# m-hamza-mughal/convofusion

Hardware: AMD Instinct MI355X
Metric: denoise-steps/sec (B=32 per GPU, 196-token latent, 1500 audio tokens, 1000-step DDPM schedule) (higher is better)
Workload: dtype f16x3 (fp16 hi/lo split operands, 3 MFMAs per product, f32 accumulate; f32-equivalent); fused cross-attention against the long (audio) memory: single-f16 operands (keys, values, queries, probabilities), f32 accumulate, in DDPM runs (operand policy 15; 1000-step DDPM golden at this shape: 2.3e-5 from; 1 GPU; configs[1]: B=32/GPU synthetic, L=196, S=(32, 1500, 32, 8, 1), 7-way guidance (denoiser batch 224), DDPM 1000-step schedule, 20 timed iterations of the hipGraph-captured loop; parallelism=batch-shard x1, one all_gather of latents

## Files before the change

convofusion_amd/csrc/cfd_dev.hip:

```cpp
#include "cfd_internal.hpp"

extern "C" int cfd_debug_stop_stage(cfd_handle c, int stage) {
  if (!c) return fail(CFD_E_ARG, "null handle");
  c->stop_stage = stage;
  return CFD_OK;
}

extern "C" int cfd_debug_weg_stop(cfd_handle c, int stop) {
  if (!c) return fail(CFD_E_ARG, "null handle");
  if (stop != 0) {
    if (!c->rt_on || !c->weg_rt_on) return fail(CFD_E_STATE, "cfd_debug_weg_stop: this handle does not evaluate on the row-tile path");
    const int l = stop / 16, k = stop % 16;
    const bool ok = stop > 0 && ((l < c->nl && k >= 1 && k <= 9 && !(l == c->nl - 1 && k < 5)) || stop == 10);
    if (!ok) return fail(CFD_E_ARG, "cfd_debug_weg_stop: %d names no launch of the reverse sweep (16 l + k, k = 1 .. 9; the top layer has no B1 .. B4; 10 = the embedding)", stop);
  }
  c->wrt.stop = stop;
  return CFD_OK;
}

static int weg_debug_buffer(Ctx* c, const char* what, float** p, size_t* n) {
  WegRtState& s = c->wrt;
  if (s.sig.empty() || !s.B) return fail(CFD_E_STATE, "'%s': no row-tile WEG evaluation has run on this handle", what);
  const size_t M = (size_t)s.B * s.L;
  int l = -1, k = -1;
// ... 27 lines not shown
    HIPCHK(hipMemcpy(p, v.data(), n * 4, hipMemcpyHostToDevice));
  }
  return CFD_OK;
}

extern "C" int cfd_debug_read(cfd_handle c, const char* what, float* dst_dev, size_t numel) {
  if (!c || !what || !dst_dev) return fail(CFD_E_ARG, "null argument");
  HIPCHK(hipSetDevice(c->cfg.device));
  if (!strcmp(what, "setup_launches")) {
    const float f = (float)c->setup_launches;
    HIPCHK(hipMemcpy(dst_dev, &f, 4, hipMemcpyHostToDevice));
    return CFD_OK;
  }
  if (!strcmp(what, "sat")) {
    unsigned int n[2] = {0, 0};
    HIPCHK(hipDeviceSynchronize());
    HIPCHK(hipMemcpy(n, c->sat.p, 8, hipMemcpyDeviceToHost));
    const float f = (float)n[0] + (float)n[1];
    HIPCHK(hipMemcpy(dst_dev, &f, 4, hipMemcpyHostToDevice));
    return CFD_OK;
  }
#if RT_STAMP
  if (!strcmp(what, "rt_ring")) {
    HIPCHK(hipDeviceSynchronize());
    if (numel * 4 < sizeof(unsigned long long) * 4 * 4096 + 8) return fail(CFD_E_ARG, "rt_ring needs %zu bytes", sizeof(unsigned long long) * 4 * 4096 + 8);
    HIPCHK(hipMemcpyFromSymbol(dst_dev, HIP_SYMBOL(g_rt_ring), sizeof(unsigned long long) * 4 * 4096, 0, hipMemcpyDeviceToDevice));
    HIPCHK(hipMemcpyFromSymbol(reinterpret_cast<char*>(dst_dev) + sizeof(unsigned long long) * 4 * 4096, HIP_SYMBOL(g_rt_seq), 4, 0, hipMemcpyDeviceToDevice));
    return CFD_OK;
  }
#endif
  if (!strcmp(what, "weg.info")) {
    if (numel < 5) return fail(CFD_E_ARG, "weg.info needs 5 floats");
    const float f[5] = {(float)c->wrt.launches, (float)c->wrt.Sp_tot, (float)c->wrt.dy_keys, (float)c->wrt.focus_large, (float)c->wrt.stop_gi};
    HIPCHK(hipMemcpy(dst_dev, f, sizeof(f), hipMemcpyHostToDevice));
    return CFD_OK;
  }
  if (!strncmp(what, "weg.", 4)) {
    float* p = nullptr;
    size_t n = 0;
    CHK(weg_debug_buffer(c, what, &p, &n));
    if (numel > n) return fail(CFD_E_ARG, "buffer '%s' holds %zu floats, asked for %zu", what, n, numel);
    HIPCHK(hipDeviceSynchronize());
    HIPCHK(hipMemcpy(dst_dev, p, numel * 4, hipMemcpyDeviceToDevice));
    return CFD_OK;
  }
  const DBuf* b = nullptr;
  if (!strcmp(what, "x")) b = &c->w->x;
  else if (!strcmp(what, "temb")) b = &c->w->temb_tab;
  else if (!strcmp(what, "ss")) b = &c->w->ss_tab;
  else if (!strcmp(what, "eps")) b = &c->w->eps;
  else if (!strcmp(what, "sc")) b = &c->w->sc;
  else if (!strcmp(what, "ssc")) b = &c->w->ssc;
  else if (!strcmp(what, "xa_stamps")) b = &c->w->xa_stamps;
  else return fail(CFD_E_ARG, "unknown buffer '%s'", what);
  if (numel * 4 > b->bytes) return fail(CFD_E_ARG, "buffer '%s' holds %zu bytes, asked for %zu", what, b->bytes, numel * 4);
  HIPCHK(hipDeviceSynchronize());
  HIPCHK(hipMemcpy(dst_dev, b->p, numel * 4, hipMemcpyDeviceToDevice));
  return CFD_OK;
}
```

convofusion_amd/csrc/cfd_internal.hpp:

```cpp
#pragma once
#include <hip/hip_runtime.h>

#include <cmath>
#include <cstdarg>
#include <cstdio>
#include <cstdlib>
#include <cstring>
#include <algorithm>
#include <map>
#include <string>
#include <vector>

#include "../../include/cfdenoise.h"
#include "../../include/cfdenoise_dev.h"
#include "gemm_sp.hpp"
#include "rows.hpp"
#include "attn_fused.hpp"
#include "xattn_fused.hpp"
#include "rowtile.hpp"


int fail(int code, const char* fmt, ...);
#define HIPCHK(expr)                                                                               \
  do {                                                                                             \
// ... 10 lines not shown

struct DBuf {
  void* p = nullptr;
  size_t bytes = 0;
  int ensure(size_t n) {
    if (n <= bytes) return CFD_OK;
    if (p) (void)hipFree(p);
    p = nullptr;
    bytes = 0;
    HIPCHK(hipMalloc(&p, n));
    bytes = n;
    return CFD_OK;
  }
  void release() {
    if (p) (void)hipFree(p);
    p = nullptr;
    bytes = 0;
  }
  template <class T> T* as() const { return reinterpret_cast<T*>(p); }
};

struct LayerW {
  DBuf wqkv_sp, bqk, wo_sp, bo2, wtb1_sp, wtb2_sp, w1_sp, w2_sp, cross_bias;
  DBuf wqk_f, wv_f, w1_f, ln_cd;
  const float *ln1g, *ln1b, *tb1g, *tb1b, *btb1, *ln2g, *ln2b, *tb2g, *tb2b, *btb2, *ln3g, *ln3b, *b1, *b2;
};

struct Problem {
  int Be = 0, L = 0, Lp = 0;
  long long M = 0;
  int U[CFD_NMEM], S[CFD_NMEM], Sp[CFD_NMEM], off[CFD_NMEM], Sp_tot = 0;
  const float* mem[CFD_NMEM];
  const int* map[CFD_NMEM];
  const uint8_t* mask[CFD_NMEM];
  int has_mask[CFD_NMEM];
  float* att[CFD_NMEM];
  int att_b0 = 0, att_nb = 0;
  bool prev_same = false;
  bool att_fused = false;
  long long att_slot[CFD_NMEM] = {0, 0, 0, 0, 0};
  int tmode = 0;
  int lv_rows = 0, lv_i0 = 0, lv_U[CFD_NMEM] = {0, 0, 0, 0, 0};
  int share_B = 0;
  int T = 1;
  int jbig = -1, nruns = 0, nlong = 0, nshort = 0;
  int run_row0[8], run_len[8], run_u[8];
  int xa_nwg = 0;
  int xa0_nwg_a = 0, xa0_nwg_b = 0;
  bool xa_flush = false;
  int xa_one = -1;
  bool xa_f16 = false;
  int xa_f16_mask = 0;
  int static_mask = 0;
  bool rt = false;
  int rt_use_inst = 0;
  unsigned char rt_inst[CFD_NMEM][RT_ARG_ROWS];
};

struct RtSave {
  float* x[CFD_MAX_LAYERS + 1][5];
  char* qk[CFD_MAX_LAYERS];
  char* vt[CFD_MAX_LAYERS];
  float* sc[CFD_MAX_LAYERS];
  float* cst[CFD_MAX_LAYERS];
  float* pre[CFD_MAX_LAYERS];
};

struct WegRtState {
  std::vector<long long> sig;
  RtSave sv;
  float *att = nullptr, *d_att = nullptr, *fws = nullptr, *dP = nullptr, *G[3] = {nullptr, nullptr, nullptr}, *dz = nullptr, *dy = nullptr,
        *dh = nullptr, *dO = nullptr, *dqkv = nullptr;
  int launches = 0;
  int T = 1;
  int stop = 0, stop_gi = -1;
  int B = 0, L = 0, Sp_tot = 0, St = 0;
  int dy_keys = 0, focus_large = 0;
};

struct Work {
  Problem pb;
  DBuf x, h_sp, qkv_sp, vts_sp, ssc, sp_sp, o_sp, u_sp, sc, p_sp, eps, sample_sp;
  DBuf ln_stat;
  DBuf n_sp[CFD_NMEM], kall_sp[CFD_NMEM], cb[CFD_NMEM], vt_all[CFD_NMEM];
  DBuf temb_tab, h1_tab, ss_tab, trows, iota, long_rows, short_rows, zero_mask;
  DBuf ca[CFD_NMEM], asq[CFD_NMEM], kbtab[CFD_NMEM], vbtab[CFD_NMEM], b_tab, b_sp, bsq, zeros512;
  DBuf xa_wgs, xa_segs, xa_stamps, xa0_wgs_a, xa0_segs_a, xa0_wgs_b, xa0_segs_b, xa_dedup, xa_one_va, xa_att_raw, xa_att_mc, xa_att_fin, xa_att_desc;
  DBuf d_step;
  bool fwd_mem_valid = false;
  int fwd_U[CFD_NMEM] = {0, 0, 0, 0, 0}, fwd_S[CFD_NMEM] = {0, 0, 0, 0, 0}, fwd_Be = 0, fwd_L = 0;
  bool fwd_att = false;
  bool fwd_mask[CFD_NMEM] = {false, false, false, false, false}, fwd_map[CFD_NMEM] = {false, false, false, false, false};
  unsigned long long fwd_wver = 0;
  DBuf rt_vt, rt_cbt[CFD_NMEM];
  DBuf k16[CFD_NMEM], v16[CFD_NMEM];
  DBuf rt_cur;
  std::vector<int32_t> tt_key;
  long long tt_wver = -1;
  int tt_mem_mask = 0;
  const float* now_ss = nullptr;
  const float* now_kb[CFD_NMEM] = {nullptr, nullptr, nullptr, nullptr, nullptr};
  const float* now_vb[CFD_NMEM] = {nullptr, nullptr, nullptr, nullptr, nullptr};
  void release() {
    DBuf* all[] = {&x, &h_sp, &qkv_sp, &vts_sp, &ssc, &sp_sp, &o_sp, &u_sp, &sc, &p_sp, &eps, &sample_sp, &temb_tab, &h1_tab, &ss_tab, &trows, &iota,
                   &long_rows, &short_rows, &zero_mask, &ln_stat, &b_tab, &b_sp, &bsq, &zeros512, &xa_wgs, &xa_segs, &xa_stamps, &xa0_wgs_a, &xa0_segs_a, &xa0_wgs_b, &xa0_segs_b, &xa_dedup, &xa_one_va, &xa_att_raw, &xa_att_mc, &xa_att_fin, &xa_att_desc, &d_step, &rt_vt, &rt_cur};
    for (DBuf* b : all) b->release();
    for (int j = 0; j < CFD_NMEM; ++j) {
      n_sp[j].release(); kall_sp[j].release(); cb[j].release(); vt_all[j].release(); ca[j].release(); asq[j].release(); kbtab[j].release();
      vbtab[j].release(); rt_cbt[j].release(); k16[j].release(); v16[j].release();
    }
  }
};

struct RunMode {
  bool weighted = false;
  int k0 = 0;
  bool edit = false;
  float* traj = nullptr;
  bool anchor = false;
  const float* anchor_ring = nullptr;
  int anchor_n = 0;
  bool tie = false;
  bool tie_final = false;
  bool replay = false;
};

struct cfd_handle_s {
  cfd_config cfg;
  int nl = 0;
  bool finalized = false;
  std::map<std::string, DBuf> raw;
  std::map<std::string, size_t> raw_numel;
  DBuf we_sp, wp_sp, we_all, be_all;
  DBuf wp_f, ln_cd_p;
  DBuf wk_all_sp[CFD_NMEM], wv_all_sp[CFD_NMEM];
  std::vector<LayerW> lw;
  int qpe_rows = 0, mpe_rows = 0;
  DBuf tsin;
  int tsin_rows = 0;
  Work wk[2];
  Work* w = &wk[0];
  long long wver = 0;
  int setup_launches = 0;
  DBuf sat;
  bool memside_in_forward = false;
  bool run_counts = false;
  DBuf acen;
  bool acen_on = false, acen_valid = false, acen_measured = false;
  int acen_hits = 0;
  float acen_tau = 0.f;
  unsigned int* sat_mem() const { return sat.as<unsigned int>() + CFD_SAT_MEM; }
  unsigned int* sat_in() const { return sat.as<unsigned int>() + CFD_SAT_IN; }
  bool want_f16 = false;
  bool hint_same_mem = false;
  bool hint_now = false;
  bool census_pending = false;
  bool rt_on = true, weg_rt_on = true, weg_graph_on = true, fused_xattn = true, l0_dedup = true, share0 = true, permute = true;
  long long rt_max_rows = 700;
// ... 131 lines not shown
}

template <int CFD_KI = 0>
__global__ void replicate_rows_kernel(float4* x, long long n4, int G) {
  const long long i = (long long)blockIdx.x * blockDim.x + threadIdx.x;
  if (i >= n4) return;
  const float4 v = x[i];
  for (int g = 1; g < G; ++g) x[(long long)g * n4 + i] = v;
}

template <int CFD_KI = 0>
__global__ void fill_f32_kernel(float* p, long long n, float v) {
  const long long i = (long long)blockIdx.x * blockDim.x + threadIdx.x;
  if (i < n) p[i] = v;
}


template <int CFD_KI = 0, int PRED = 0>
__global__ void sched_step_kernel(const float* eps, const float* noise, float* x, size_t n, StepCoef c, int kind, int clip, float* x0_out) {
  const size_t i = (size_t)blockIdx.x * blockDim.x + threadIdx.x;
  if (i >= n) return;
  const float e = eps[i], xv = x[i];
  const float x0 = step_x0_of<PRED>(c, clip, xv, e);
  if (x0_out) x0_out[i] = x0;
  float prev = (kind == 0) ? c.c0 * x0 + c.cx * xv : c.c0 * x0 + c.cx * step_eps_of<PRED>(c, xv, e);
  if (c.use_noise != 0.f) prev = prev + c.sigma * noise[i];
  x[i] = prev;
}
template <int CFD_KI = 0, int PRED = 0>
__global__ void dpmpp_step_kernel(const float* eps, const float* m_prev, float* x, float* x0_out, size_t n, StepCoef c) {
  const size_t i = (size_t)blockIdx.x * blockDim.x + threadIdx.x;
  if (i >= n) return;
  const float xv = x[i];
  const float x0 = step_x0_of<PRED>(c, 0, xv, eps[i]);
  const float m1 = c.order == 2.0f ? m_prev[i] : 0.f;
  x0_out[i] = x0;
  x[i] = dpmpp_prev(c, xv, x0, m1);
}
template <int CFD_KI = 0>
__global__ void add_noise_kernel(const float* x0, const float* noise, float* out, size_t n, float sa, float sb) {
  const size_t i = (size_t)blockIdx.x * blockDim.x + threadIdx.x;
  if (i < n) out[i] = sa * x0[i] + sb * noise[i];
}

int to_sp(Ctx* c, const float* src, long long R, int K, DBuf& dst, long long dst_rows = -1);
int enqueue_to_split(Ctx* c, int cls, hipStream_t st, const float* src, char* dst, long long R, int K, long long ld_src, long long ld_dst, unsigned int* sat);
int ln_fold_weight(Ctx* c, const float* W, int R, int K, const float* gamma, const float* beta, DBuf& tmp, DBuf& dst_sp, float* cvec, float* dvec);
int build_xattn_worklist(Ctx* c, const cfd_memory mem[CFD_NMEM], bool one_key);
int build_xattn_layer0_lists(Ctx* c, const cfd_memory mem[CFD_NMEM]);
int setup_att_fused(Ctx* c);
int setup_problem(Ctx* c, int Be, int L, const cfd_memory mem[CFD_NMEM], float* const att[CFD_NMEM], int tmode, int T);
int build_time_tables(Ctx* c, const int32_t* trows_host, int T, hipStream_t st);
int enqueue_time_tables(Ctx* c, int T, hipStream_t st);
int prepare_static_memside(Ctx* c, hipStream_t st, int dynamic_mask, bool want_att, bool reuse = false);
int enqueue_memside(Ctx* c, hipStream_t st);
int enqueue_rows(Ctx* c, hipStream_t st, int row0, int nrows);
int enqueue_rows_rt(Ctx* c, hipStream_t st, const RtSave* sv = nullptr);
int enqueue_denoise(Ctx* c, hipStream_t st);
int run_gemm_plain_f32(Ctx* c, int cls, const GemmArgs& a, const EpiF32& e, int nb, int nz, hipStream_t st);
int enqueue_philox_fill(float* out, int B, int per_utt, uint64_t seed, uint32_t step, uint32_t utt0, uint32_t stream_id, float scale, hipStream_t st);
int enqueue_linear_act(const float* x, long long n_rows, int K, const float* W, const float* b, int N, int act, float* out, hipStream_t st);
```

convofusion_amd/csrc/cfd_problem.hip:

```cpp
#include "cfd_internal.hpp"

struct XaRow {
  int xrow;
  int inst[CFD_NMEM];
  int aux;
  int one;
  int att;
};

static void make_xattn_worklist(const Problem& p, const std::vector<XaRow>& rows, int mem_mask, std::vector<XaWg>& wgs, std::vector<XaSeg>& segs,
                                size_t& n_active, bool& has_flush) {
  const int L = p.L, nqt = (L + 15) / 16;
  wgs.clear(); segs.clear(); n_active = 0;
  int order[CFD_NMEM], n_mem = 0, n_online = 0;
  for (int j = 0; j < CFD_NMEM; ++j)
    if ((mem_mask >> j) & 1) order[n_mem++] = j;
  if (n_mem == 0 || rows.empty()) return;
  std::stable_sort(order, order + n_mem, [&](int a, int b) { return p.Sp[a] > p.Sp[b]; });
  for (int oi = 0; oi < n_mem; ++oi) n_online += p.Sp[order[oi]] > XA_KEYS;
  const int jg = order[0];
  std::vector<int> inst_group(p.U[jg], -1);
  std::vector<std::vector<int>> groups;
  for (size_t r = 0; r < rows.size(); ++r) {
    int& g = inst_group[rows[r].inst[jg]];
// ... 329 lines not shown
  CHK(c->w->sample_sp.ensure((size_t)M * CFD_LAT * 4));
  for (int j = 0; j < CFD_NMEM; ++j) {
    const size_t rows = (size_t)p.U[j] * p.Sp[j];
    CHK(c->w->n_sp[j].ensure(rows * CFD_D * 4));
    CHK(c->w->kall_sp[j].ensure(rows * nl * CFD_D * 4));
    CHK(c->w->cb[j].ensure(rows * (nl + 1) * 4));
    CHK(c->w->vt_all[j].ensure(rows * nl * CFD_D * 4));
  }
  if (c->w->temb_tab.bytes < (size_t)T * CFD_D * 4 || c->w->ss_tab.bytes < (size_t)T * nl * 2 * 2 * CFD_D * 4) {
    c->w->tt_key.clear();
    c->w->tt_mem_mask = 0;
  }
  CHK(c->w->temb_tab.ensure((size_t)T * CFD_D * 4));
  CHK(c->w->h1_tab.ensure((size_t)T * CFD_D * 4));
  CHK(c->w->ss_tab.ensure((size_t)T * nl * 2 * 2 * CFD_D * 4));
  CHK(c->w->trows.ensure((size_t)T * 4));
  return CFD_OK;
}

int build_time_tables(Ctx* c, const int32_t* trows_host, int T, hipStream_t st) {
  for (int i = 0; i < T; ++i)
    if (trows_host[i] < 0 || trows_host[i] >= c->tsin_rows)
      return fail(CFD_E_ARG, "timestep %d outside the sinusoid table (0..%d)", trows_host[i], c->tsin_rows - 1);
  HIPCHK(hipMemcpyAsync(c->w->trows.p, trows_host, (size_t)T * 4, hipMemcpyHostToDevice, st));
  Work* w = c->w;
  const bool same = w->tt_wver == c->wver && (int)w->tt_key.size() == T && std::equal(w->tt_key.begin(), w->tt_key.end(), trows_host);
  if (same) return CFD_OK;
  w->tt_key.assign(trows_host, trows_host + T);
  w->tt_wver = c->wver;
  w->tt_mem_mask = 0;
  c->setup_launches += 2 + 2 * c->nl;
  return enqueue_time_tables(c, T, st);
}

int enqueue_time_tables(Ctx* c, int T, hipStream_t st) {
  const int ry = T < 64 ? T : 64;
  const float* W1 = rawp(c, "time_embedding.linear_1.weight");
  const float* b1 = rawp(c, "time_embedding.linear_1.bias");
  const float* W2 = rawp(c, "time_embedding.linear_2.weight");
  const float* b2 = rawp(c, "time_embedding.linear_2.bias");
  const int NE = c->nl * 2 * 2 * CFD_D;
  LAUNCH(CFD_PROF_OTHER, small_linear_kernel<>, dim3(CFD_D / 4, ry), dim3(256), st, c->tsin.as<float>(), c->w->trows.as<int>(),
         (long long)CFD_D, W1, b1, c->w->h1_tab.as<float>(), (long long)CFD_D, T, CFD_D, 0, 1);
  LAUNCH(CFD_PROF_OTHER, small_linear_kernel<>, dim3(CFD_D / 4, ry), dim3(256), st, c->w->h1_tab.as<float>(), (const int*)nullptr,
         (long long)CFD_D, W2, b2, c->w->temb_tab.as<float>(), (long long)CFD_D, T, CFD_D, 0, 0);
  for (int tb = 0; tb < c->nl * 2; ++tb) {
    LAUNCH(CFD_PROF_OTHER, small_linear_kernel<>, dim3(2 * CFD_D / 4, ry), dim3(256), st, c->w->temb_tab.as<float>(), (const int*)nullptr,
           (long long)CFD_D, c->we_all.as<float>() + (size_t)tb * 2 * CFD_D * CFD_D, c->be_all.as<float>() + (size_t)tb * 2 * CFD_D,
           c->w->ss_tab.as<float>() + (size_t)tb * 2 * CFD_D, (long long)NE, T, 2 * CFD_D, 1, 2);
  }
  return CFD_OK;
}

int prepare_static_memside(Ctx* c, hipStream_t st, int dynamic_mask, bool want_att, bool reuse) {
  Problem& p = c->w->pb;
  const int nl = c->nl;
  const long long ROWB = CFD_D * 4;
  p.static_mask = 0;
  for (int j = 0; j < CFD_NMEM; ++j) {
    const long long rows = (long long)p.U[j] * p.Sp[j];
    LAUNCH(CFD_PROF_OTHER, fill_f32_kernel<>, dim3((unsigned)((rows + 255) / 256)), dim3(256), st, c->w->cb[j].as<float>() + (size_t)nl * rows, rows, 1.0f);
  }
  if (c->w->zeros512.bytes == 0) {
    CHK(c->w->zeros512.ensure(CFD_D * 4));
    HIPCHK(hipMemsetAsync(c->w->zeros512.p, 0, CFD_D * 4, st));
  }
  if (dynamic_mask) p.rt = false;
  if (p.xa_one >= 0 && ((dynamic_mask >> p.xa_one) & 1)) {
    cfd_memory mem[CFD_NMEM];
    memset(mem, 0, sizeof(mem));
    for (int j = 0; j < CFD_NMEM; ++j) {
      mem[j].data = p.mem[j]; mem[j].U = p.U[j]; mem[j].S = p.S[j]; mem[j].row_map = p.map[j];
      mem[j].key_padding_mask = p.has_mask[j] ? p.mask[j] : nullptr;
    }
    CHK(build_xattn_worklist(c, mem, false));
  }
  const bool fused = p.rt || (c->fused_xattn && p.xa_nwg > 0 && !want_att);
  if (!fused || p.tmode != 0) { p.xa_f16 = false; return CFD_OK; }
  const int T = p.T;
  if (c->w->b_tab.bytes < (size_t)T * CFD_D * 4 || c->w->b_sp.bytes < (size_t)T * CFD_D * 4 || c->w->bsq.bytes < (size_t)T * 4)
    c->w->tt_mem_mask = 0;
  CHK(c->w->b_tab.ensure((size_t)T * CFD_D * 4));
  CHK(c->w->b_sp.ensure((size_t)T * CFD_D * 4));
  CHK(c->w->bsq.ensure((size_t)T * 4));
  if (c->w->tt_mem_mask == 0) {
    c->w->tt_mem_mask = 0;
    LAUNCH(CFD_PROF_OTHER, temb_center_kernel<>, dim3((unsigned)((T + 3) / 4)), dim3(256), st, c->w->temb_tab.as<float>(), T, c->w->b_tab.as<float>(),
           c->w->b_sp.as<char>(), c->w->bsq.as<float>());
    c->setup_launches += 1;
  }
  for (int j = 0; j < CFD_NMEM; ++j) {
    if ((dynamic_mask >> j) & 1) continue;
    const int rows = p.U[j] * p.Sp[j];
    const int NK = nl * CFD_D + 32;
    CHK(c->w->ca[j].ensure((size_t)rows * nl * 4));
    CHK(c->w->asq[j].ensure((size_t)rows * 4));
    if (c->w->kbtab[j].bytes < (size_t)T * NK * 4 || c->w->vbtab[j].bytes < (size_t)T * nl * CFD_D * 4) c->w->tt_mem_mask &= ~(1 << j);
    CHK(c->w->kbtab[j].ensure((size_t)T * NK * 4));
    CHK(c->w->vbtab[j].ensure((size_t)T * nl * CFD_D * 4));
    const bool have_tb = (c->w->tt_mem_mask >> j) & 1;
    MemCenterArgs ma{p.mem[j], p.U[j], p.S[j], p.Sp[j], rawp(c, "condition_embedding.weight") + (size_t)j * CFD_D, rawp(c, "mem_pos.pe"),
                     c->w->n_sp[j].as<char>(), c->w->asq[j].as<float>(), c->sat_mem()};
    if (!reuse) LAUNCH(CFD_PROF_ROWS, mem_center_kernel<>, dim3((unsigned)((rows + 3) / 4)), dim3(256), st, ma);
    if (!reuse) {
      GemmArgs a = gemm_args();
      a.X[0] = c->wk_all_sp[j].as<char>(); a.ldx[0] = ROWB; a.I[0] = NK; a.Iclamp[0] = NK; a.kt[0] = CFD_D / 32;
      a.Y = c->w->n_sp[j].as<char>(); a.ldy = ROWB; a.J = rows; a.Jclamp = rows;
      a.super_i = 8; a.super_j = 8;
      EpiMemK e{c->w->kall_sp[j].as<char>(), (long long)rows, c->w->ca[j].as<float>(), nl * CFD_D, nl, p.mask[j], p.S[j], p.Sp[j], c->sat_mem()};
      CHK((run_gemm<MODE_PLAIN>(c, CFD_PROF_GEMM_MEM, a, e, 1, 1, st)));
    }
    if (!reuse) {
      GemmArgs a = gemm_args();
      a.X[0] = c->w->n_sp[j].as<char>(); a.ldx[0] = ROWB; a.I[0] = rows; a.Iclamp[0] = rows; a.kt[0] = CFD_D / 32;
      a.Y = c->wv_all_sp[j].as<char>(); a.ldy = ROWB; a.J = nl * CFD_D; a.Jclamp = nl * CFD_D;
      a.super_i = 8; a.super_j = 8;
      EpiMemV e{c->w->vt_all[j].as<char>(), p.Sp[j], p.U[j], c->sat_mem()};
      CHK((run_gemm<MODE_PLAIN>(c, CFD_PROF_GEMM_MEM, a, e, 1, 1, st)));
    }
    if (!have_tb) {
      GemmArgs a = gemm_args();
      a.X[0] = c->wk_all_sp[j].as<char>(); a.ldx[0] = ROWB; a.I[0] = NK; a.Iclamp[0] = NK; a.kt[0] = CFD_D / 32;
      a.Y = c->w->b_sp.as<char>(); a.ldy = ROWB; a.J = T; a.Jclamp = T;
      EpiF32 e;
      memset(&e, 0, sizeof(e));
      e.out = c->w->kbtab[j].as<float>(); e.ldo = NK;
      CHK(run_gemm_plain_f32(c, CFD_PROF_GEMM_MEM, a, e, 1, 1, st));
    }
    if (!have_tb) {
      GemmArgs a = gemm_args();
      a.X[0] = c->wv_all_sp[j].as<char>(); a.ldx[0] = ROWB; a.I[0] = nl * CFD_D; a.Iclamp[0] = nl * CFD_D; a.kt[0] = CFD_D / 32;
      a.Y = c->w->b_sp.as<char>(); a.ldy = ROWB; a.J = T; a.Jclamp = T;
      EpiF32 e;
      memset(&e, 0, sizeof(e));
      e.out = c->w->vbtab[j].as<float>(); e.ldo = nl * CFD_D;
      CHK(run_gemm_plain_f32(c, CFD_PROF_GEMM_MEM, a, e, 1, 1, st));
      c->w->tt_mem_mask |= 1 << j;
      c->setup_launches += 2;
    }
    p.static_mask |= 1 << j;
  }
  if (p.xa_f16 && (p.rt || p.static_mask != (1 << CFD_NMEM) - 1)) p.xa_f16 = false;
  if (p.xa_f16) {
    for (int j = 0; j < CFD_NMEM; ++j) {
      if (!((p.xa_f16_mask >> j) & 1)) continue;
      const long long tiles = (long long)nl * p.U[j] * (p.Sp[j] / XA_KEYS), chunks = tiles * 2048;
      CHK(c->w->v16[j].ensure((size_t)tiles * 32768));
      LAUNCH(CFD_PROF_ROWS, xa_pack16_kernel<>, dim3((unsigned)((chunks + 255) / 256)), dim3(256), st, c->w->vt_all[j].as<char>(), c->w->v16[j].as<char>(), chunks, p.Sp[j], 0);
      CHK(c->w->k16[j].ensure((size_t)tiles * 32768));
      LAUNCH(CFD_PROF_ROWS, xa_pack16_kernel<>, dim3((unsigned)((chunks + 255) / 256)), dim3(256), st, c->w->kall_sp[j].as<char>(), c->w->k16[j].as<char>(), chunks, p.Sp[j], 1);
    }
  }
  if (p.xa_one >= 0 && !p.rt) {
    const int j = p.xa_one;
    const long long n = (long long)nl * p.U[j] * CFD_D;
    CHK(c->w->xa_one_va.ensure((size_t)n * 4));
    LAUNCH(CFD_PROF_ROWS, one_key_va_kernel<>, dim3((unsigned)((n + 255) / 256)), dim3(256), st, c->w->vt_all[j].as<char>(), n, p.Sp[j], c->w->xa_one_va.as<float>());
  }
  if (p.rt) {
    for (int j = 0; j < CFD_NMEM; ++j) {
      const long long rows = (long long)p.U[j] * p.Sp[j];
      CHK(c->w->rt_cbt[j].ensure((size_t)T * (nl + 1) * rows * 4));
      MemScaleTabArgs a{c->w->n_sp[j].as<char>(), c->w->asq[j].as<float>(), rows, c->w->b_tab.as<float>(), c->w->bsq.as<float>(), c->w->ca[j].as<float>(),
                        c->w->kbtab[j].as<float>() + (size_t)nl * CFD_D, (long long)(nl * CFD_D + 32), nl, c->w->rt_cbt[j].as<float>()};
      LAUNCH(CFD_PROF_ROWS, mem_scale_table_kernel<>, dim3((unsigned)((rows + 3) / 4), (unsigned)T), dim3(256), st, a);
    }
  }
  return CFD_OK;
}

int enqueue_memside(Ctx* c, hipStream_t st) {
  const Problem& p = c->w->pb;
  if (p.rt) return CFD_OK;
  const int nl = c->nl;
  const int* dstep = p.tmode ? c->w->d_step.as<int>() + 1 : c->w->d_step.as<int>();
  const long long ROWB = CFD_D * 4;
  const dim3 blk(256);
  {
    MemScaleAllArgs g;
    memset(&g, 0, sizeof(g));
    int nwg = 0;
    for (int j = 0; j < CFD_NMEM; ++j) {
      if (!((p.static_mask >> j) & 1)) continue;
      const long long rows = (long long)p.U[j] * p.Sp[j];
      const int NK = nl * CFD_D + 32;
      g.m[g.n] = MemScaleArgs{c->w->n_sp[j].as<char>(), c->w->asq[j].as<float>(), rows, c->w->b_tab.as<float>(), c->w->bsq.as<float>(), c->w->ca[j].as<float>(),
                              c->w->kbtab[j].as<float>() + (size_t)nl * CFD_D, (long long)NK, dstep, nl, c->w->cb[j].as<float>() + (size_t)nl * rows,
                              c->w->cb[j].as<float>()};
      g.first[g.n] = nwg;
      nwg += (int)((rows + 3) / 4);
      ++g.n;
    }
    g.first[g.n] = nwg;
    if (g.n > 0) LAUNCH(CFD_PROF_ROWS, mem_scale_all_kernel<>, dim3((unsigned)nwg), blk, st, g);
  }
  for (int j = 0; j < CFD_NMEM; ++j) {
    if ((p.static_mask >> j) & 1) continue;
    const long long rows = (long long)p.U[j] * p.Sp[j];
    if (p.tmode == 2) {
      MemPrepLevelArgs la{p.mem[j], p.lv_U[j], p.U[j], p.S[j], p.Sp[j], c->w->temb_tab.as<float>(), p.lv_i0,
                          rawp(c, "condition_embedding.weight") + (size_t)j * CFD_D, rawp(c, "mem_pos.pe"), c->w->n_sp[j].as<char>()};
      LAUNCH(CFD_PROF_ROWS, mem_prep_level_kernel<>, dim3((unsigned)((rows + 3) / 4)), blk, st, la);
      continue;
    }
    MemPrepArgs a{p.mem[j], p.U[j], p.S[j], p.Sp[j], c->w->temb_tab.as<float>(), dstep, p.tmode,
                  rawp(c, "condition_embedding.weight") + (size_t)j * CFD_D, rawp(c, "mem_pos.pe"), c->w->n_sp[j].as<char>()};
    LAUNCH(CFD_PROF_ROWS, mem_prep_kernel<>, dim3((unsigned)((rows + 3) / 4)), blk, st, a);
  }
  for (int j = 0; j < CFD_NMEM; ++j) {
    if ((p.static_mask >> j) & 1) continue;
    const int rows = p.U[j] * p.Sp[j];
    c->memside_in_forward = true;
    {
      GemmArgs a = gemm_args();
      a.X[0] = c->wk_all_sp[j].as<char>(); a.ldx[0] = ROWB; a.I[0] = nl * CFD_D + 32; a.Iclamp[0] = nl * CFD_D + 32; a.kt[0] = CFD_D / 32;
      a.Y = c->w->n_sp[j].as<char>(); a.ldy = ROWB; a.J = rows; a.Jclamp = rows;
      a.super_i = 8; a.super_j = 8;
      EpiMemK e{c->w->kall_sp[j].as<char>(), (long long)rows, c->w->cb[j].as<float>(), nl * CFD_D, nl, p.mask[j], p.S[j], p.Sp[j], c->sat_mem()};
      CHK((run_gemm<MODE_PLAIN>(c, CFD_PROF_GEMM_MEM, a, e, 1, 1, st)));
    }
    {
      GemmArgs a = gemm_args();
      a.X[0] = c->w->n_sp[j].as<char>(); a.ldx[0] = ROWB; a.I[0] = rows; a.Iclamp[0] = rows; a.kt[0] = CFD_D / 32;
      a.Y = c->wv_all_sp[j].as<char>(); a.ldy = ROWB; a.J = nl * CFD_D; a.Jclamp = nl * CFD_D;
      a.super_i = 8; a.super_j = 8;
      EpiMemV e{c->w->vt_all[j].as<char>(), p.Sp[j], p.U[j], c->sat_mem()};
      CHK((run_gemm<MODE_PLAIN>(c, CFD_PROF_GEMM_MEM, a, e, 1, 1, st)));
    }
  }

  return CFD_OK;
// ... 3 lines not shown
```

convofusion_amd/csrc/cfd_sample.hip:

```cpp
#include "cfd_internal.hpp"

static void ddpm_coef(const float* ac, int T, int n_inf, int t, StepCoef* o) {
  const int prev_t = t - T / n_inf;
  const float ap_t = ac[t];
  const float ap_prev = prev_t >= 0 ? ac[prev_t] : 1.0f;
  const float bp_t = 1.0f - ap_t, bp_prev = 1.0f - ap_prev;
  const float cur_alpha = ap_t / ap_prev;
  const float cur_beta = 1.0f - cur_alpha;
  o->sb = sqrtf(bp_t);
  o->sa = sqrtf(ap_t);
  o->c0 = (sqrtf(ap_prev) * cur_beta) / bp_t;
  o->cx = sqrtf(cur_alpha) * bp_prev / bp_t;
  float var = bp_prev / bp_t * cur_beta;
  if (var < 1e-20f) var = 1e-20f;
  o->sigma = t > 0 ? sqrtf(var) : 0.0f;
  o->use_noise = t > 0 ? 1.0f : 0.0f;
  o->order = o->r0inv = 0.f;
}
static void ddim_coef(const float* ac, int T, int n_inf, int t, float eta, int set_alpha_to_one, StepCoef* o) {
  const int prev_t = t - T / n_inf;
  const float ap_t = ac[t];
  const float ap_prev = prev_t >= 0 ? ac[prev_t] : (set_alpha_to_one ? 1.0f : ac[0]);
  const float bp_t = 1.0f - ap_t, bp_prev = 1.0f - ap_prev;
  const float var = (bp_prev / bp_t) * (1.0f - ap_t / ap_prev);
// ... 165 lines not shown
  }
  const long long n4 = (long long)s.B * s.L * CFD_LAT / 4;
  const dim3 grid((unsigned)std::min<long long>((n4 + 255) / 256, 256)), block(256);
  return with_step_inst(m.weighted, m.traj != nullptr, s.prediction_type, [&](auto inst, const char* name) {
    LAUNCH_AS(CFD_PROF_OTHER, name, inst.kernel, grid, block, st, inst.args(cw, m.traj));
    return (int)CFD_OK;
  });
}

static int host_row_map(const cfd_memory& mem, int rows, const char* name, std::vector<int>& out) {
  out.resize((size_t)rows);
  if (mem.row_map) {
    HIPCHK(hipMemcpy(out.data(), mem.row_map, (size_t)rows * 4, hipMemcpyDeviceToHost));
    return CFD_OK;
  }
  if (mem.U != rows) return fail(CFD_E_ARG, "memory %s: U = %d != G * B = %d without a row_map", name, mem.U, rows);
  for (int r = 0; r < rows; ++r) out[r] = r;
  return CFD_OK;
}

static int setup_preamble(Ctx* c) {
  HIPCHK(hipSetDevice(c->cfg.device));
  c->hint_now = c->hint_same_mem = false;
  return settle_deferred_census(c);
}

static int check_scheduler_tables(const cfd_sample_args& s, const char* who) {
  if (!s.alphas_cumprod || s.num_train_timesteps < 1 || s.num_inference_steps < 1 || s.num_inference_steps > s.num_train_timesteps)
    return fail(CFD_E_ARG, "bad scheduler tables");
  if (s.timesteps && (s.num_timesteps < 1 || s.num_timesteps > s.num_train_timesteps)) return fail(CFD_E_ARG, "bad num_timesteps");
  if (!s.timesteps && s.scheduler == 0 && s.num_train_timesteps % s.num_inference_steps)
    return fail(CFD_E_ARG, "%s: DDPM: num_inference_steps = %d does not divide num_train_timesteps = %d: the loop's timestep table for such "
                           "counts differs between diffusers releases (unpinned); pass the scheduler's table in cfd_sample_args.timesteps",
                who, s.num_inference_steps, s.num_train_timesteps);
  return CFD_OK;
}

static void trim_zero_weight_chunks(Ctx* c, const cfd_sample_args& s) {
  if (s.skip_zero_weight_chunks)
    while (c->sargs.G > 1 && s.guidance_weight[c->sargs.G - 1] == 0.0f) c->sargs.G -= 1;
}

static int upload_run_tables(Ctx* c, const cfd_sample_args& s, int N, int k0, hipStream_t st, std::vector<StepCoef>* coef_out = nullptr) {
  const int n_inf = s.num_inference_steps, T = s.num_train_timesteps, ratio = T / n_inf;
  std::vector<int32_t> ts(N);
  std::vector<StepCoef> coef(N);
  for (int i = 0; i < N; ++i) ts[i] = s.timesteps ? s.timesteps[i] : (N - 1 - i) * ratio + (s.scheduler == 1 ? s.steps_offset : 0);
  CHK(step_coefficients(s.scheduler, s.alphas_cumprod, T, n_inf, ts.data(), N, s.eta, s.set_alpha_to_one, coef.data(), k0));
  CHK(c->coef.ensure((size_t)N * sizeof(StepCoef)));
  HIPCHK(hipMemcpyAsync(c->coef.p, coef.data(), (size_t)N * sizeof(StepCoef), hipMemcpyHostToDevice, st));
  HIPCHK(hipMemsetAsync(c->w->d_step.p, 0, 16, st));
  CHK(sat_begin(c, st));
  CHK(build_time_tables(c, ts.data(), N, st));
  CHK(prepare_static_memside(c, st, s.dynamic_memory_mask, false));
  HIPCHK(hipStreamSynchronize(st));
  if (coef_out) coef_out->swap(coef);
  return CFD_OK;
}

static int weighted_chunks(Ctx* c, const float* wtab, int prune, int N, bool keep_last, cfd_memory mem_in[CFD_NMEM], int keep_idx[8],
                           hipStream_t st) {
  const cfd_sample_args& s = c->sargs;
  const int B = s.B, G = s.G;
  const size_t n = (size_t)N * B * 8;
  for (size_t e = 0; e < n; ++e)
    if (e % 8 != 0 && !std::isfinite(wtab[e]))
      return fail(CFD_E_ARG, "weights[%zu][%zu][%zu] is not finite", e / 8 / B, e / 8 % B, e % 8);
  bool keep[8] = {true, false, false, false, false, false, false, false};
  for (int k = 1; k < G; ++k) {
    keep[k] = !prune || (keep_last && k == G - 1);
    for (size_t r = 0; r < (size_t)N * B && !keep[k]; ++r) keep[k] = wtab[r * 8 + k] != 0.0f;
  }
  int ge = 0;
  for (int k = 0; k < 8; ++k) keep_idx[k] = (k < G && keep[k]) ? ge++ : -1;
  CHK(c->wtab.ensure(n * sizeof(float)));
  HIPCHK(hipMemcpyAsync(c->wtab.p, wtab, n * sizeof(float), hipMemcpyHostToDevice, st));
  HIPCHK(hipStreamSynchronize(st));
  c->sargs.G = ge;
  if (ge == G) return CFD_OK;
  const int Be = G * B, Bc = ge * B;
  std::vector<int> hm, cm(Bc);
  for (int j = 0; j < CFD_NMEM; ++j) {
    CHK(host_row_map(mem_in[j], Be, MEM_NAMES[j], hm));
    for (int k = 0; k < G; ++k)
      if (keep_idx[k] >= 0)
        for (int u = 0; u < B; ++u) cm[(size_t)keep_idx[k] * B + u] = hm[(size_t)k * B + u];
    CHK(c->perm_map[j].ensure((size_t)Be * 4));
    HIPCHK(hipMemcpy(c->perm_map[j].p, cm.data(), (size_t)Bc * 4, hipMemcpyHostToDevice));
    mem_in[j].row_map = c->perm_map[j].as<int32_t>();
  }
  return CFD_OK;
}

static int upload_keep_mask(Ctx* c, const std::vector<uint8_t>& hkeep, size_t n, hipStream_t st) {
  CHK(c->ekeep.ensure(n));
  if (!hkeep.empty()) HIPCHK(hipMemcpyAsync(c->ekeep.p, hkeep.data(), n, hipMemcpyHostToDevice, st));
  else HIPCHK(hipMemsetAsync(c->ekeep.p, 0, n, st));
  return CFD_OK;
}

struct BeginExt {
  const char* opener = "cfd_sample_begin";
  const float* weights = nullptr;
  int prune = 0;
  int* chunks_evaluated = nullptr;
  const cfd_edit_args* edit = nullptr;
  float* traj = nullptr;
// ... 751 lines not shown
  if (n < 0 || a->run_pos + n > a->run_iters || (b && b->run_pos + n > b->run_iters))
    return fail(CFD_E_ARG, "run has %d of %d iterations done; cannot run %d more", a->run_pos, a->run_iters, n);
  HIPCHK(hipSetDevice(a->cfg.device));
  hipStream_t st = a->run_stream;
  if (b) {
    HIPCHK(hipEventRecord(b->weg_ev, b->run_stream));
    HIPCHK(hipStreamWaitEvent(st, b->weg_ev, 0));
  }
  const int Bs = b ? sa.B : sa.B / 2;
  const long long rows = (long long)Bs * sa.L;
  const dim3 blk(256);
  const long long gy = (rows + 31) / 32;
  if (gy > 65535) return fail(CFD_E_ARG, "too many rows for one launch (%lld)", rows);
  auto project = [&](const float* lat, float* spk) {
    (void)enqueue_linear_act(lat, rows, CFD_LAT, pr->w1, pr->b1, pr->hidden, 1, pr->tmp, st);
    (void)enqueue_linear_act((const float*)pr->tmp, rows, pr->hidden, pr->w2, pr->b2, pr->out_dim, 1, spk, st);
  };
  const float* lat_a = a->latents.as<float>();
  const float* lat_b = b ? b->latents.as<float>() : lat_a + rows * CFD_LAT;
  for (int i = 0; i < n; ++i) {
    project(lat_b, pr->spk_a);
    project(lat_a, pr->spk_b);
    HIPCHK(hipGetLastError());
    HIPCHK(hipGraphLaunch(a->gexec, st));
    if (b) HIPCHK(hipGraphLaunch(b->gexec, st));
  }
  a->run_pos += n;
  if (b) {
    b->run_pos += n;
    HIPCHK(hipEventRecord(a->weg_ev, st));
    HIPCHK(hipStreamWaitEvent(b->run_stream, a->weg_ev, 0));
  }
  return CFD_OK;
}

extern "C" int cfd_sample_position(cfd_handle c) { return (c && c->run_open) ? c->run_pos : -1; }

extern "C" int cfd_sample_read(cfd_handle c, float* out, int close) {
  if (!c || !out) return fail(CFD_E_ARG, "null argument");
  if (!c->run_open) return fail(CFD_E_STATE, "no sampling run open");
  HIPCHK(hipSetDevice(c->cfg.device));
  const size_t lat_bytes = (size_t)c->sargs.B * c->sargs.L * CFD_LAT * 4;
  if (c->run.tie && !c->run.tie_final && c->run_pos == c->run_iters) {
    const long long n8 = (long long)c->sargs.B * c->sargs.L * (CFD_LAT / 8);
    hipLaunchKernelGGL(tie_copy_kernel<>, dim3((unsigned)((n8 + 255) / 256)), dim3(256), 0, c->run_stream, c->latents.as<float>(),
                       c->etie.as<int32_t>(), n8);
    HIPCHK(hipGetLastError());
    c->run.tie_final = true;
  }
  HIPCHK(hipMemcpyAsync(out, c->latents.p, lat_bytes, hipMemcpyDeviceToDevice, c->run_stream));
  HIPCHK(hipStreamSynchronize(c->run_stream));
  CHK(settle_deferred_census(c));
  if (c->run_counts) CHK(check_saturation(c, "sampling run (the per-step projections of a memory)"));
  if (close) c->run_open = false;
  return CFD_OK;
}

extern "C" int cfd_scheduler_step_pred(cfd_handle c, int scheduler, const float* ac, int T, int n_inf, int t, int clip, float eta,
                                       int set_alpha_to_one, int prediction_type, const float* model_output, const float* noise,
                                       float* sample_inout, size_t numel, float* pred_original_sample, void* stream) {
  if (!c || !ac || !model_output || !sample_inout || t < 0 || t >= T || n_inf < 1) return fail(CFD_E_ARG, "bad argument");
  if (prediction_type != 0 && prediction_type != 1)
    return fail(CFD_E_ARG, "cfd_scheduler_step_pred: prediction_type = %d is not 0 (epsilon) or 1 (sample)", prediction_type);
  if (scheduler == 3 && prediction_type != 0)
    return fail(CFD_E_ARG, "cfd_scheduler_step_pred: DDIM inversion needs prediction_type = 0 (epsilon)");
  if (scheduler != 0 && scheduler != 1 && scheduler != 3)
    return fail(CFD_E_ARG, "cfd_scheduler_step[_pred]: scheduler must be 0 (DDPM), 1 (DDIM) or 3 (DDIM inversion); DPM-Solver++ steps go "
                           "through cfd_dpmsolver_step[_pred]");
  if (scheduler == 3 && (eta != 0.f || clip))
    return fail(CFD_E_ARG, "cfd_scheduler_step[_pred]: DDIM inversion needs eta = 0 and clip_sample = 0 (got %g, %d)", (double)eta, clip);
  HIPCHK(hipSetDevice(c->cfg.device));
  StepCoef k;
  memset(&k, 0, sizeof(k));
  if (scheduler == 0) ddpm_coef(ac, T, n_inf, t, &k);
  else if (scheduler == 3) ddim_inverse_coef(ac, T, n_inf, t, set_alpha_to_one, &k);
  else ddim_coef(ac, T, n_inf, t, eta, set_alpha_to_one, &k);
  if (k.use_noise != 0.f && !noise) return fail(CFD_E_ARG, "this step adds noise: pass the N(0,1) draw");
  const dim3 grid((unsigned)((numel + 255) / 256)), block(256);
  with_pred(prediction_type, [&](auto pred) {
    hipLaunchKernelGGL((sched_step_kernel<0, decltype(pred)::value>), grid, block, 0, (hipStream_t)stream, model_output, noise, sample_inout, numel, k,
                       scheduler, clip, pred_original_sample);
  });
  HIPCHK(hipGetLastError());
  return CFD_OK;
}

extern "C" int cfd_scheduler_step(cfd_handle c, int scheduler, const float* ac, int T, int n_inf, int t, int clip, float eta,
                                  int set_alpha_to_one, const float* model_output, const float* noise, float* sample_inout,
                                  size_t numel, float* pred_original_sample, void* stream) {
  return cfd_scheduler_step_pred(c, scheduler, ac, T, n_inf, t, clip, eta, set_alpha_to_one, 0, model_output, noise, sample_inout, numel,
                                 pred_original_sample, stream);
}

extern "C" int cfd_dpmsolver_step_pred(cfd_handle c, const float* ac, int T, int t, int prev_t, int t_prev_model, int prediction_type,
                                       const float* model_output, const float* m_prev, float* sample_inout, float* x0_out, size_t numel,
                                       void* stream) {
  if (!c || !ac || !model_output || !sample_inout || !x0_out) return fail(CFD_E_ARG, "null argument");
  if (prediction_type != 0 && prediction_type != 1)
    return fail(CFD_E_ARG, "cfd_dpmsolver_step_pred: prediction_type = %d is not 0 (epsilon) or 1 (sample)", prediction_type);
  if (t < 1 || t >= T || prev_t < 0 || prev_t >= t || t_prev_model >= T || (t_prev_model >= 0 && t_prev_model <= t))
    return fail(CFD_E_ARG, "cfd_dpmsolver_step[_pred]: need T > t_prev_model > t > prev_t >= 0 (t_prev_model = -1: first order), t >= 1 "
                           "(got %d, %d, %d, T = %d)", t_prev_model, t, prev_t, T);
  if (t_prev_model >= 0 && !m_prev) return fail(CFD_E_ARG, "a second-order step reads the previous step's x0: pass m_prev");
  HIPCHK(hipSetDevice(c->cfg.device));
  StepCoef k;
  dpmpp_coef(ac, t, prev_t, t_prev_model, &k);
  const dim3 grid((unsigned)((numel + 255) / 256)), block(256);
// ... 139 lines not shown
```

convofusion_amd/csrc/rows.hpp:

```cpp
#pragma once
#include "cfd_common.hpp"

struct LnArgs {
  const float* x;
  char* out;
  long long M;
  const float* g;
  const float* b;
  int adaln;
  const float* ss;
  long long ss_tstride;
  const int* d_step;
  int tmode;
  int L;
  int trow0;
};

template <int CFD_KI = 0>
__global__ void __launch_bounds__(256) ln_rows_kernel(const LnArgs a) {
  const int lane = threadIdx.x & 63;
  const long long row = (long long)blockIdx.x * 4 + (threadIdx.x >> 6);
  if (row >= a.M) return;
  const float* xr = a.x + row * CFD_D + lane * 8;
  const long long trow = a.tmode ? (a.trow0 + row / a.L) : (a.d_step ? (long long)(*a.d_step) : 0);
// ... 128 lines not shown
  const int* d_step;
  int nl;
  float* rs;
  float* cbk;
};

struct MemScaleAllArgs {
  MemScaleArgs m[CFD_NMEM];
  int first[CFD_NMEM + 1];
  int n;
};

__device__ __forceinline__ void mem_scale_rows(const MemScaleArgs& a, long long row, int lane);

template <int CFD_KI = 0>
__global__ void __launch_bounds__(256) mem_scale_all_kernel(const MemScaleAllArgs g) {
  int k = 0;
#pragma unroll
  for (int q = 1; q < CFD_NMEM; ++q)
    if (q < g.n && (int)blockIdx.x >= g.first[q]) k = q;
  MemScaleArgs a = g.m[0];
#pragma unroll
  for (int q = 1; q < CFD_NMEM; ++q)
    if (k == q) a = g.m[q];
  int first = 0;
#pragma unroll
  for (int q = 1; q < CFD_NMEM; ++q)
    if (k == q) first = g.first[q];
  const long long row = (long long)((int)blockIdx.x - first) * 4 + (threadIdx.x >> 6);
  if (row >= a.rows) return;
  mem_scale_rows(a, row, threadIdx.x & 63);
}

__device__ __forceinline__ void mem_scale_rows(const MemScaleArgs& a, long long row, int lane) {
  const int t = *a.d_step;
  const char* ap = a.a_sp + row * (CFD_D * 4) + (size_t)(lane >> 2) * 128 + (lane & 3) * 16;
  const spx8 h = *reinterpret_cast<const spx8*>(ap);
  const spx8 l = *reinterpret_cast<const spx8*>(ap + 64);
  const float* bp = a.btab + (long long)t * CFD_D + lane * 8;
  const float4 b0 = *reinterpret_cast<const float4*>(bp), b1 = *reinterpret_cast<const float4*>(bp + 4);
  const int ll = min(lane, a.nl - 1);
  const float asq = a.asq[row], bsq = a.bsq[t];
  const float ca = a.ca[(long long)ll * a.rows + row], cbb = a.cbb[(long long)t * a.cbb_tstride + ll];
  __builtin_amdgcn_sched_barrier(0);
  const float bv[8] = {b0.x, b0.y, b0.z, b0.w, b1.x, b1.y, b1.z, b1.w};
  float dot = 0.f;
#pragma unroll
  for (int e = 0; e < 8; ++e) dot += ((float)h[e] + (float)l[e]) * bv[e];
  dot = wave_sum(dot);
  const float var = (asq + 2.0f * dot + bsq) * (1.0f / CFD_D);
  const float rstd = 1.0f / sqrtf(var + 1e-5f);
  if (lane == 0) a.rs[row] = rstd;
  if (lane < a.nl) a.cbk[(long long)lane * a.rows + row] = rstd * (ca + cbb);
}

template <int CFD_KI = 0>
__global__ void __launch_bounds__(256) temb_center_kernel(const float* temb, int T, float* b, char* b_sp, float* bsq) {
  const int lane = threadIdx.x & 63;
  const int row = blockIdx.x * 4 + (threadIdx.x >> 6);
  if (row >= T) return;
  float v[8];
  float sum = 0.f;
#pragma unroll
  for (int e = 0; e < 8; ++e) { v[e] = temb[(long long)row * CFD_D + lane * 8 + e]; sum += v[e]; }
  const float mean = wave_sum(sum) * (1.0f / CFD_D);
  float ss = 0.f;
#pragma unroll
  for (int e = 0; e < 8; ++e) { v[e] -= mean; ss += v[e] * v[e]; b[(long long)row * CFD_D + lane * 8 + e] = v[e]; }
  ss = wave_sum(ss);
  sp_store8(b_sp + (long long)row * (CFD_D * 4), lane * 8, v);
  if (lane == 0) bsq[row] = ss;
}

#define SM_MAX_CHUNKS 4
struct SoftmaxArgs {
  const float* sc;
  char* P;
  long long ld;
  long long rows;
  int rows_per_b;
  int nseg;
  int off[CFD_NMEM], S[CFD_NMEM], Sp[CFD_NMEM];
  const uint8_t* mask[CFD_NMEM];
  int has_mask[CFD_NMEM];
  const int* map[CFD_NMEM];
  float* att[CFD_NMEM];
  int layer, nl;
  int skip_seg;
  const uint8_t* skip_rows;
};

__device__ __forceinline__ void softmax_store(const SoftmaxArgs& a, int g, int b, int l, char* prow, int c0, float* v) {
  const int S = a.S[g];
  sp_store8_keep_nan(prow, a.off[g] + c0, v);
  if (a.att[g]) {
    float* att = a.att[g] + (((long long)b * a.nl + a.layer) * a.rows_per_b + l) * S;
#pragma unroll
    for (int e = 0; e < 8; ++e)
      if (c0 + e < S) att[c0 + e] = v[e];
  }
}

template <int CFD_KI = 0>
__global__ void __launch_bounds__(256) softmax_rows_kernel(const SoftmaxArgs a) {
  const int lane = threadIdx.x & 63;
  const long long row = (long long)blockIdx.x * 4 + (threadIdx.x >> 6);
// ... 942 lines not shown
```

Before: 82.49 denoise-steps/s (32-utterance batches, summed over GPUs).

## Precompute per-timestep memory-key dot table for static memories at run setup

At sampling-run setup, a new kernel computes the dot product of every static memory key row with every timestep's centered embedding and stores a T x rows table. Each denoise step then reads one table row instead of recomputing a 512-wide dot per key row to get the LayerNorm rstd and per-layer scales. This removes per-step reads of the key activations in the memory-side scaling kernel. In exchange it adds a large one-time table (T times total key rows floats) and a setup kernel, and the per-step kernel now does a strided gather plus a serial loop over layers per thread.

```diff
diff --git a/convofusion_amd/csrc/cfd_dev.hip b/convofusion_amd/csrc/cfd_dev.hip
--- a/convofusion_amd/csrc/cfd_dev.hip
+++ b/convofusion_amd/csrc/cfd_dev.hip
@@ -103,6 +103,12 @@
   else if (!strcmp(what, "sc")) b = &c->w->sc;
   else if (!strcmp(what, "ssc")) b = &c->w->ssc;
   else if (!strcmp(what, "xa_stamps")) b = &c->w->xa_stamps;
+  else if (!strcmp(what, "b_tab")) b = &c->w->b_tab;
+  else if (!strcmp(what, "bsq")) b = &c->w->bsq;
+  else if (strlen(what) == 3 && !strncmp(what, "cb", 2) && what[2] >= '0' && what[2] < '0' + CFD_NMEM) b = &c->w->cb[what[2] - '0'];
+  else if (strlen(what) == 3 && !strncmp(what, "ca", 2) && what[2] >= '0' && what[2] < '0' + CFD_NMEM) b = &c->w->ca[what[2] - '0'];
+  else if (strlen(what) == 4 && !strncmp(what, "asq", 3) && what[3] >= '0' && what[3] < '0' + CFD_NMEM) b = &c->w->asq[what[3] - '0'];
+  else if (strlen(what) == 6 && !strncmp(what, "kbtab", 5) && what[5] >= '0' && what[5] < '0' + CFD_NMEM) b = &c->w->kbtab[what[5] - '0'];
   else return fail(CFD_E_ARG, "unknown buffer '%s'", what);
   if (numel * 4 > b->bytes) return fail(CFD_E_ARG, "buffer '%s' holds %zu bytes, asked for %zu", what, b->bytes, numel * 4);
   HIPCHK(hipDeviceSynchronize());
diff --git a/convofusion_amd/csrc/cfd_internal.hpp b/convofusion_amd/csrc/cfd_internal.hpp
--- a/convofusion_amd/csrc/cfd_internal.hpp
+++ b/convofusion_amd/csrc/cfd_internal.hpp
@@ -86,6 +86,8 @@
   bool xa_f16 = false;
   int xa_f16_mask = 0;
   int static_mask = 0;
+  bool key_tab = false;
+  long long key_tab_ld = 0, key_tab_off[CFD_NMEM] = {0, 0, 0, 0, 0};
   bool rt = false;
   int rt_use_inst = 0;
   unsigned char rt_inst[CFD_NMEM][RT_ARG_ROWS];
@@ -127,6 +129,7 @@
   bool fwd_mask[CFD_NMEM] = {false, false, false, false, false}, fwd_map[CFD_NMEM] = {false, false, false, false, false};
   unsigned long long fwd_wver = 0;
   DBuf rt_vt, rt_cbt[CFD_NMEM];
+  DBuf dtab;
   DBuf k16[CFD_NMEM], v16[CFD_NMEM];
   DBuf rt_cur;
   std::vector<int32_t> tt_key;
@@ -137,7 +140,7 @@
   const float* now_vb[CFD_NMEM] = {nullptr, nullptr, nullptr, nullptr, nullptr};
   void release() {
     DBuf* all[] = {&x, &h_sp, &qkv_sp, &vts_sp, &ssc, &sp_sp, &o_sp, &u_sp, &sc, &p_sp, &eps, &sample_sp, &temb_tab, &h1_tab, &ss_tab, &trows, &iota,
-                   &long_rows, &short_rows, &zero_mask, &ln_stat, &b_tab, &b_sp, &bsq, &zeros512, &xa_wgs, &xa_segs, &xa_stamps, &xa0_wgs_a, &xa0_segs_a, &xa0_wgs_b, &xa0_segs_b, &xa_dedup, &xa_one_va, &xa_att_raw, &xa_att_mc, &xa_att_fin, &xa_att_desc, &d_step, &rt_vt, &rt_cur};
+                   &long_rows, &short_rows, &zero_mask, &ln_stat, &b_tab, &b_sp, &bsq, &zeros512, &xa_wgs, &xa_segs, &xa_stamps, &xa0_wgs_a, &xa0_segs_a, &xa0_wgs_b, &xa0_segs_b, &xa_dedup, &xa_one_va, &xa_att_raw, &xa_att_mc, &xa_att_fin, &xa_att_desc, &d_step, &rt_vt, &rt_cur, &dtab};
     for (DBuf* b : all) b->release();
     for (int j = 0; j < CFD_NMEM; ++j) {
       n_sp[j].release(); kall_sp[j].release(); cb[j].release(); vt_all[j].release(); ca[j].release(); asq[j].release(); kbtab[j].release();
@@ -375,7 +378,7 @@
 int setup_problem(Ctx* c, int Be, int L, const cfd_memory mem[CFD_NMEM], float* const att[CFD_NMEM], int tmode, int T);
 int build_time_tables(Ctx* c, const int32_t* trows_host, int T, hipStream_t st);
 int enqueue_time_tables(Ctx* c, int T, hipStream_t st);
-int prepare_static_memside(Ctx* c, hipStream_t st, int dynamic_mask, bool want_att, bool reuse = false);
+int prepare_static_memside(Ctx* c, hipStream_t st, int dynamic_mask, bool want_att, bool reuse = false, bool key_table = false);
 int enqueue_memside(Ctx* c, hipStream_t st);
 int enqueue_rows(Ctx* c, hipStream_t st, int row0, int nrows);
 int enqueue_rows_rt(Ctx* c, hipStream_t st, const RtSave* sv = nullptr);
diff --git a/convofusion_amd/csrc/cfd_problem.hip b/convofusion_amd/csrc/cfd_problem.hip
--- a/convofusion_amd/csrc/cfd_problem.hip
+++ b/convofusion_amd/csrc/cfd_problem.hip
@@ -405,11 +405,12 @@
   return CFD_OK;
 }
 
-int prepare_static_memside(Ctx* c, hipStream_t st, int dynamic_mask, bool want_att, bool reuse) {
+int prepare_static_memside(Ctx* c, hipStream_t st, int dynamic_mask, bool want_att, bool reuse, bool key_table) {
   Problem& p = c->w->pb;
   const int nl = c->nl;
   const long long ROWB = CFD_D * 4;
   p.static_mask = 0;
+  p.key_tab = false;
   for (int j = 0; j < CFD_NMEM; ++j) {
     const long long rows = (long long)p.U[j] * p.Sp[j];
     LAUNCH(CFD_PROF_OTHER, fill_f32_kernel<>, dim3((unsigned)((rows + 255) / 256)), dim3(256), st, c->w->cb[j].as<float>() + (size_t)nl * rows, rows, 1.0f);
@@ -510,6 +511,32 @@
     CHK(c->w->xa_one_va.ensure((size_t)n * 4));
     LAUNCH(CFD_PROF_ROWS, one_key_va_kernel<>, dim3((unsigned)((n + 255) / 256)), dim3(256), st, c->w->vt_all[j].as<char>(), n, p.Sp[j], c->w->xa_one_va.as<float>());
   }
+  if (key_table && !p.rt && p.static_mask) {
+    MemDotAllArgs g;
+    memset(&g, 0, sizeof(g));
+    long long ld = 0;
+    int nwg = 0;
+    for (int j = 0; j < CFD_NMEM; ++j) {
+      p.key_tab_off[j] = ld;
+      if ((p.static_mask >> j) & 1) ld += (long long)p.U[j] * p.Sp[j];
+    }
+    CHK(c->w->dtab.ensure((size_t)T * ld * 4));
+    for (int j = 0; j < CFD_NMEM; ++j) {
+      if (!((p.static_mask >> j) & 1)) continue;
+      const long long rows = (long long)p.U[j] * p.Sp[j];
+      g.m[g.n] = MemDotArgs{c->w->n_sp[j].as<char>(), rows, c->w->dtab.as<float>() + p.key_tab_off[j]};
+      g.first[g.n] = nwg;
+      nwg += (int)((rows + 15) / 16);
+      ++g.n;
+    }
+    g.first[g.n] = nwg;
+    g.btab = c->w->b_tab.as<float>();
+    g.T = T;
+    g.ld = ld;
+    LAUNCH(CFD_PROF_ROWS, mem_dot_table_kernel<>, dim3((unsigned)nwg), dim3(256), st, g);
+    p.key_tab_ld = ld;
+    p.key_tab = true;
+  }
   if (p.rt) {
     for (int j = 0; j < CFD_NMEM; ++j) {
       const long long rows = (long long)p.U[j] * p.Sp[j];
@@ -529,7 +556,26 @@
   const int* dstep = p.tmode ? c->w->d_step.as<int>() + 1 : c->w->d_step.as<int>();
   const long long ROWB = CFD_D * 4;
   const dim3 blk(256);
-  {
+  if (p.key_tab) {
+    MemScaleStepArgs g;
+    memset(&g, 0, sizeof(g));
+    int nwg = 0;
+    for (int j = 0; j < CFD_NMEM; ++j) {
+      if (!((p.static_mask >> j) & 1)) continue;
+      const long long rows = (long long)p.U[j] * p.Sp[j];
+      const int NK = nl * CFD_D + 32;
+      g.m[g.n] = MemScaleArgs{nullptr, c->w->asq[j].as<float>(), rows, nullptr, c->w->bsq.as<float>(), c->w->ca[j].as<float>(),
+                              c->w->kbtab[j].as<float>() + (size_t)nl * CFD_D, (long long)NK, dstep, nl, c->w->cb[j].as<float>() + (size_t)nl * rows,
+                              c->w->cb[j].as<float>()};
+      g.D[g.n] = c->w->dtab.as<float>() + p.key_tab_off[j];
+      g.first[g.n] = nwg;
+      nwg += (int)((rows + 255) / 256);
+      ++g.n;
+    }
+    g.first[g.n] = nwg;
+    g.ld = p.key_tab_ld;
+    if (g.n > 0) LAUNCH(CFD_PROF_ROWS, mem_scale_step_kernel<>, dim3((unsigned)nwg), blk, st, g);
+  } else {
     MemScaleAllArgs g;
     memset(&g, 0, sizeof(g));
     int nwg = 0;
diff --git a/convofusion_amd/csrc/cfd_sample.hip b/convofusion_amd/csrc/cfd_sample.hip
--- a/convofusion_amd/csrc/cfd_sample.hip
+++ b/convofusion_amd/csrc/cfd_sample.hip
@@ -241,7 +241,7 @@
   HIPCHK(hipMemsetAsync(c->w->d_step.p, 0, 16, st));
   CHK(sat_begin(c, st));
   CHK(build_time_tables(c, ts.data(), N, st));
-  CHK(prepare_static_memside(c, st, s.dynamic_memory_mask, false));
+  CHK(prepare_static_memside(c, st, s.dynamic_memory_mask, false, false, true));
   HIPCHK(hipStreamSynchronize(st));
   if (coef_out) coef_out->swap(coef);
   return CFD_OK;
@@ -1099,7 +1099,11 @@
   HIPCHK(hipStreamSynchronize(c->run_stream));
   CHK(settle_deferred_census(c));
   if (c->run_counts) CHK(check_saturation(c, "sampling run (the per-step projections of a memory)"));
-  if (close) c->run_open = false;
+  if (close) {
+    c->run_open = false;
+    c->w->pb.key_tab = false;
+    c->w->dtab.release();
+  }
   return CFD_OK;
 }
 
diff --git a/convofusion_amd/csrc/rows.hpp b/convofusion_amd/csrc/rows.hpp
--- a/convofusion_amd/csrc/rows.hpp
+++ b/convofusion_amd/csrc/rows.hpp
@@ -204,6 +204,103 @@
   const float rstd = 1.0f / sqrtf(var + 1e-5f);
   if (lane == 0) a.rs[row] = rstd;
   if (lane < a.nl) a.cbk[(long long)lane * a.rows + row] = rstd * (ca + cbb);
+}
+
+struct MemDotArgs {
+  const char* a_sp;
+  long long rows;
+  float* D;
+};
+struct MemDotAllArgs {
+  MemDotArgs m[CFD_NMEM];
+  int first[CFD_NMEM + 1];
+  int n;
+  const float* btab;
+  int T;
+  long long ld;
+};
+
+template <int CFD_KI = 0>
+__global__ void __launch_bounds__(256) mem_dot_table_kernel(const MemDotAllArgs g) {
+  int k = 0;
+#pragma unroll
+  for (int q = 1; q < CFD_NMEM; ++q)
+    if (q < g.n && (int)blockIdx.x >= g.first[q]) k = q;
+  MemDotArgs a = g.m[0];
+#pragma unroll
+  for (int q = 1; q < CFD_NMEM; ++q)
+    if (k == q) a = g.m[q];
+  int first = 0;
+#pragma unroll
+  for (int q = 1; q < CFD_NMEM; ++q)
+    if (k == q) first = g.first[q];
+  const int lane = threadIdx.x & 63;
+  const long long row0 = ((long long)((int)blockIdx.x - first) * 4 + (threadIdx.x >> 6)) * 4;
+  if (row0 >= a.rows) return;
+  float av[4][8];
+#pragma unroll
+  for (int r = 0; r < 4; ++r) {
+    const char* ap = a.a_sp + (row0 + r) * (CFD_D * 4) + (size_t)(lane >> 2) * 128 + (lane & 3) * 16;
+    const spx8 h = *reinterpret_cast<const spx8*>(ap);
+    const spx8 l = *reinterpret_cast<const spx8*>(ap + 64);
+#pragma unroll
+    for (int e = 0; e < 8; ++e) av[r][e] = (float)h[e] + (float)l[e];
+  }
+  float keep[4] = {0.f, 0.f, 0.f, 0.f};
+  for (int t = 0; t < g.T; ++t) {
+    const float* bp = g.btab + (long long)t * CFD_D + lane * 8;
+    const float4 b0 = *reinterpret_cast<const float4*>(bp), b1 = *reinterpret_cast<const float4*>(bp + 4);
+    const float bv[8] = {b0.x, b0.y, b0.z, b0.w, b1.x, b1.y, b1.z, b1.w};
+#pragma unroll
+    for (int r = 0; r < 4; ++r) {
+      float dot = 0.f;
+#pragma unroll
+      for (int e = 0; e < 8; ++e) dot += av[r][e] * bv[e];
+      dot = wave_sum(dot);
+      if (lane == (t & 63)) keep[r] = dot;
+    }
+    if ((t & 63) == 63 || t + 1 == g.T) {
+      const int tl = (t & ~63) + lane;
+      if (tl <= t) *reinterpret_cast<float4*>(a.D + (long long)tl * g.ld + row0) = make_float4(keep[0], keep[1], keep[2], keep[3]);
+    }
+  }
+}
+
+struct MemScaleStepArgs {
+  MemScaleArgs m[CFD_NMEM];
+  const float* D[CFD_NMEM];
+  int first[CFD_NMEM + 1];
+  int n;
+  long long ld;
+};
+
+template <int CFD_KI = 0>
+__global__ void __launch_bounds__(256) mem_scale_step_kernel(const MemScaleStepArgs g) {
+  int k = 0;
+#pragma unroll
+  for (int q = 1; q < CFD_NMEM; ++q)
+    if (q < g.n && (int)blockIdx.x >= g.first[q]) k = q;
+  MemScaleArgs a = g.m[0];
+  const float* D = g.D[0];
+#pragma unroll
+  for (int q = 1; q < CFD_NMEM; ++q)
+    if (k == q) { a = g.m[q]; D = g.D[q]; }
+  int first = 0;
+#pragma unroll
+  for (int q = 1; q < CFD_NMEM; ++q)
+    if (k == q) first = g.first[q];
+  const long long row = (long long)((int)blockIdx.x - first) * 256 + threadIdx.x;
+  if (row >= a.rows) return;
+  const int t = *a.d_step;
+  const float dot = D[(long long)t * g.ld + row];
+  const float asq = a.asq[row], bsq = a.bsq[t];
+  const float var = (asq + 2.0f * dot + bsq) * (1.0f / CFD_D);
+  const float rstd = 1.0f / sqrtf(var + 1e-5f);
+  a.rs[row] = rstd;
+  for (int l = 0; l < a.nl; ++l) {
+    const float ca = a.ca[(long long)l * a.rows + row], cbb = a.cbb[(long long)t * a.cbb_tstride + l];
+    a.cbk[(long long)l * a.rows + row] = rstd * (ca + cbb);
+  }
 }
 
 template <int CFD_KI = 0>
```

New measurement: 82.54 denoise-steps/s (32-utterance batches, summed over GPUs), median of 3. No clear change (+0.1%).
